# kcat/openal-soft

Hardware: AMD Instinct MI355X
Metric: mixed voices/sec @48kHz 1024-sample update, HRTF stereo; fraction of HBM roofline (higher is better)
Workload: dtype f32

## Files before the change

include/oalgpu.h:

```cpp
#ifndef OALGPU_H
#define OALGPU_H

#include <stddef.h>
#include <stdint.h>

#ifdef __cplusplus
extern "C" {
#endif
#if defined(__GNUC__)
#pragma GCC visibility push(default)
#endif

#define OALGPU_BUFFER_LINE_SIZE 1024
#define OALGPU_MAX_RESAMPLER_PADDING 48
#define OALGPU_MAX_RESAMPLER_EDGE 24
#define OALGPU_HRTF_HISTORY_LENGTH 64
#define OALGPU_HRIR_LENGTH 128
#define OALGPU_MAX_SENDS 6
#define OALGPU_MAX_OUTPUT_CHANNELS 32
#define OALGPU_MAX_AMBI_CHANNELS 25
#define OALGPU_MIXER_FRAC_BITS 16

typedef enum oalgpu_error {
    OALGPU_OK = 0,
// ... 91 lines not shown
    int32_t  hrtf;
    uint32_t max_voices;
    uint32_t max_buffers;
    uint32_t voices_per_group;
    uint32_t flags;
} oalgpu_context_desc;
#define OALGPU_CTX_FIR_VALU 1u
#define OALGPU_CTX_PROFILE  2u
#define OALGPU_CTX_STREAM_ROWS 8u
#define OALGPU_CTX_APPLY_IN_VOICE_KERNEL 16u
#define OALGPU_CTX_FUSED_REDUCE 32u
#define OALGPU_CTX_RESIDENT 64u
#define OALGPU_CTX_SLICE_LINES 128u
#define OALGPU_CTX_WAVE_PAIRS 256u
#define OALGPU_CTX_ROW_SLICES 512u
#define OALGPU_CTX_SERIAL   4u

int  oalgpu_context_create(const oalgpu_context_desc *desc, oalgpu_context **out);
void oalgpu_context_destroy(oalgpu_context *ctx);

int oalgpu_hrtf_load_mhr(oalgpu_context *ctx, const void *data, size_t size);
int oalgpu_hrtf_load_store(oalgpu_context *ctx, uint32_t sample_rate, uint32_t ir_size, const float *field_distance,
    const uint8_t *field_evcount, uint32_t num_fields, const uint16_t *elev_azcount, const uint16_t *elev_iroffset,
    uint32_t num_elevs, const float *coeffs, const uint8_t *delays, uint32_t num_irs);
typedef struct oalgpu_hrtf_info {
    uint32_t sample_rate, ir_size, num_fields, num_elevs, num_irs;
} oalgpu_hrtf_info;
int oalgpu_hrtf_info_get(oalgpu_context *ctx, oalgpu_hrtf_info *out);
int oalgpu_hrtf_raw(oalgpu_context *ctx, float *field_distance, uint8_t *field_evcount,
    uint16_t *elev_azcount, uint16_t *elev_iroffset, float *coeffs, uint8_t *delays);
// ... 352 lines not shown
```

openal-soft_amd/csrc/api.hip:

```cpp
#include "api_context.hpp"
namespace oalgpu {

thread_local std::string gLastError;

int Fail(int code, const std::string &msg)
{
    gLastError = msg;
    return code;
}

void ParkResidentContexts(int device);

int UseDevice(int device)
{
    int count = 0;
    if(hipGetDeviceCount(&count) != hipSuccess || count <= 0)
        return Fail(OALGPU_ERR_NO_DEVICE, "no HIP device available (the product has no CPU path)");
    if(device < 0 || device >= count) return Fail(OALGPU_ERR_INVALID, "device ordinal out of range");
    HIP_TRY(hipSetDevice(device));
    ParkResidentContexts(device);
    return OALGPU_OK;
}

}
// ... 212 lines not shown
    HIP_TRY(c->partHrtf.alloc(L.hrtf ? groups * (kLine + kHrirLen) * 2 : 0)); L.partHrtf = c->partHrtf.p;
    HIP_TRY(c->partHrtf2.alloc(c->useWave && L.hrtf ? groups * (kLine + kHrirLen) * 2 : 0));
    c->partHrtfBuf[0] = c->partHrtf.p; c->partHrtfBuf[1] = c->partHrtf2.p;
    HIP_TRY(c->bus.alloc(BusFloats(L))); HIP_TRY(c->bus.zero()); L.bus = c->bus.p;
    if(desc->flags & OALGPU_CTX_PROFILE)
    {
        HIP_TRY(c->phaseTimes.alloc(nv * 16)); HIP_TRY(c->phaseTimes.zero());
        c->prof.times = c->phaseTimes.p;
    }
    L.hrtfOld = nullptr; L.hrtfTgt = nullptr;

    HIP_TRY(c->dSplit.alloc(L.numDry)); HIP_TRY(c->dSplit.zero());
    HIP_TRY(c->dSplit2.alloc(L.numDry)); HIP_TRY(c->dSplit2.zero());
    HIP_TRY(c->carryBuf.alloc(size_t{kLine + kHrirLen} * 2)); HIP_TRY(c->carryBuf.zero());
    HIP_TRY(c->postArrived.alloc(1)); HIP_TRY(c->postArrived.zero());
    HIP_TRY(c->dHfScale.alloc(L.numDry)); HIP_TRY(c->dHfScale.zero());
    HIP_TRY(c->dCoeffs.alloc(size_t{L.numDry} * kHrirLen * 2)); HIP_TRY(c->dCoeffs.zero());
    HIP_TRY(c->dTemp.alloc(size_t{L.numDry} * kLine + (kLine + kHrirLen) * 2));
    if(L.rows8) SetRowsGroups(c.get());
    *out = c.release();
    return OALGPU_OK;
}

static void DetachForDestroy(oalgpu_context *ctx);

void oalgpu_context_destroy(oalgpu_context *ctx)
{
    if(!ctx) return;
    (void)UseDevice(ctx->desc.device);
    if(ctx->attachedTo || !ctx->attached.empty()) DetachForDestroy(ctx);
// ... 85 lines not shown
        }
    out[0] = st[0][0]; out[1] = st[0][1]; out[2] = st[1][1]; out[3] = st[2][2];
}

static int PostDirectHrtfFused(oalgpu_context *c, hipStream_t s, uint32_t samples_to_do, hipEvent_t evDone, bool resident = false)
{
    const DeviceLayout &L = c->L;
    float *left = L.bus + size_t{L.numDry} * kLine;
    SplitterState *spIn = c->dSplitCur ? c->dSplit2.p : c->dSplit.p, *spOut = c->dSplitCur ? c->dSplit.p : c->dSplit2.p;
    const uint32_t postEpoch = c->postEpoch + L.numDry;
    const uint32_t seg = ((samples_to_do + 63u) / 64u) | 1u;
    if(c->runPowerSeg != seg) { SplitterRunPowers(c->dSplitCoeff, seg, c->runPower); c->runPowerSeg = seg; }
    const uint32_t slot = c->outNext % oalgpu_context::kIoSlots;
    const bool ring = c->outRing && c->outFlags;
    const uint32_t outTarget = c->outArrivedTotal + PostResidentFirGroups();
    auto &R = c->res;
    if(resident)
    {
        c->reduceHeld = false;
        LaunchPostResident(s, left, left + kLine, L.bus, L.numDry, L.bus + BusAccumOffset(L), c->carryBuf.p, spIn, spOut, c->dHfScale.p, c->dCoeffs.p,
            c->dIrSize, samples_to_do, c->dTemp.p, c->postArrived.p, postEpoch, c->runPower, evDone, ring ? c->outHost[slot] : nullptr,
            ring ? c->outFlags + size_t{slot} * 16 : nullptr, c->outSeq + 1u, R.counters.p, R.hostFlags, (R.posts + 1u) * R.redGroups,
            (R.posts + 1u) * R.firGroups, R.posts + 1u);
        HIP_TRY(hipGetLastError());
        ++R.posts;
    }
    else if(c->reduceHeld)
    {
        c->reduceHeld = false;
        if(!c->reducedCount.p) { HIP_TRY(c->reducedCount.alloc(1)); HIP_TRY(c->reducedCount.zero()); }
        const uint32_t reducedEpoch = c->reducedEpoch + ReducePostReduceGroups(c->heldL);
        LaunchReducePostFused(s, c->heldL, CarrySource(c, c->carryAccum && L.hrtf), left, left + kLine, L.bus, L.numDry, L.bus + BusAccumOffset(L),
            c->carryBuf.p, spIn, spOut, c->dHfScale.p, c->dCoeffs.p, c->dIrSize, samples_to_do, c->dTemp.p, c->postArrived.p, postEpoch,
            c->runPower, evDone, ring ? c->outHost[slot] : nullptr, ring ? c->outFlags + size_t{slot} * 16 : nullptr, c->outSeq + 1u,
            c->outArrived.p, outTarget, c->reducedCount.p, reducedEpoch);
        HIP_TRY(hipGetLastError());
        c->reducedEpoch = reducedEpoch;
        if(ring) c->outArrivedTotal = outTarget;
    }
    else
    {
        LaunchPostDirectHrtfFused(s, left, left + kLine, L.bus, L.numDry, L.bus + BusAccumOffset(L), c->carryBuf.p, spIn, spOut,
            c->dHfScale.p, c->dCoeffs.p, c->dIrSize, samples_to_do, c->dTemp.p, c->postArrived.p, postEpoch, c->runPower, evDone,
            ring ? c->outHost[slot] : nullptr, ring ? c->outFlags + size_t{slot} * 16 : nullptr, c->outSeq + 1u, c->outArrived.p, outTarget);
        HIP_TRY(hipGetLastError());
        if(ring) c->outArrivedTotal = outTarget;
    }
    c->postEpoch = postEpoch;
    if(ring) c->outSlotSeq[slot] = ++c->outSeq;
    c->outRingWritten = ring;
    c->dSplitCur ^= 1u;
    c->carryInBuf = true;
    return OALGPU_OK;
}

int JoinPost(oalgpu_context *c)
{
    if(!c->postPending) return OALGPU_OK;
    HIP_TRY(hipStreamWaitEvent(c->stream, c->lastPostEvent ? c->lastPostEvent : c->evPostDone, 0));
// ... 787 lines not shown
```

openal-soft_amd/csrc/api_context.hpp:

```cpp
#pragma once
#include "../../include/oalgpu.h"
#ifdef OALGPU_MEASUREMENT
#include "../../tools/measure/oalgpu_measure.h"
#endif

#include <hip/hip_runtime.h>
#include <hip/hip_ext.h>
#include <rccl/rccl.h>
#include <dlfcn.h>
#include <fcntl.h>
#include <sys/mman.h>
#include <sys/stat.h>
#include <unistd.h>

#include <algorithm>
#include <atomic>
#include <chrono>
#include <functional>
#include <thread>
#include <cstdio>
#include <cstdlib>
#include <cstring>
#include <memory>
#include <mutex>
// ... 169 lines not shown
    DevBuf<float> cfState;
    uint32_t distLines{0};
    DevBuf<uint32_t> distDelays;
    DevBuf<float> distGains, distHist;
    DevBuf<unsigned char> pcm;
    DevBuf<float> hFieldDist, hCoeffs;
    DevBuf<uint8_t> hEvCount, hDelays;
    DevBuf<uint16_t> hAzCount, hIrOffset;
    DevBuf<SplitterState> dSplit, dSplit2;
    uint32_t dSplitCur{0};
    DevBuf<float> carryBuf;
    float dSplitCoeff{0.0f};
    float runPower[4]{1.0f, 0.0f, 1.0f, 1.0f};
    uint32_t runPowerSeg{0};
    DevBuf<uint32_t> postArrived;
    uint32_t postEpoch{0};
    const ParamRecord *nextRecs{nullptr};
    const int32_t *nextMap{nullptr};
    const float *nextRows{nullptr};
    bool carryInBuf{false};
    DevBuf<float> dHfScale, dCoeffs, dTemp;
    uint32_t dIrSize{0};
    bool directSet{false};
    DevBuf<ParamRecord> paramDev;
    std::vector<ParamRecord> paramHost;
    DevBuf<VoiceInitRecord> initDev;
    std::vector<VoiceInitRecord> initPending;
    struct CbVoice {
        uint32_t voice{0}; int32_t buffer{-1}; uint32_t frameBytes{4}, capacityFrames{0};
        oalgpu_callback_fn fn{nullptr}; void *user{nullptr};
// ... 119 lines not shown
```

openal-soft_amd/csrc/kernels.hpp:

```cpp
#pragma once
#include <hip/hip_runtime.h>
#include <stdint.h>

#include "dev_hrtf.hpp"
#include "dev_mix.hpp"
#include "dev_resample.hpp"
#include "dev_voice.hpp"
#include "../host/limiter_params.hpp"
#include "../host/uhj_params.hpp"
#include "../host/stabilizer_params.hpp"
#include "../host/crossfeed_params.hpp"

namespace oalgpu {

enum VoiceFlagBits : uint32_t {
    kFlagFading = 1u << 0,
    kFlagHasHrtf = 1u << 1,
    kFlagDirectFilter = 1u << 2,
    kFlagHrtfDirty = 1u << 3,
    kFlagAmbiScale = 1u << 4,
    kFlagNfc = 1u << 5,
    kFlagQueue = 1u << 7,
    kFlagDelayed = 1u << 6,
    kFlagSendFilterShift = 8
// ... 199 lines not shown
void LaunchMixDirectHrtf(hipStream_t s, bool exact, float *left, float *right, const float *in, uint32_t nch,
    float *accum, SplitterState *splitters, const float *hfscales, const float *chanCoeffs, uint32_t irsize,
    uint32_t n, float *temp);
void LaunchBiquadDual(hipStream_t s, BiquadState *f0, BiquadState *f1, const float *src, float *dst, uint32_t n);
void LaunchGetCoeffs(hipStream_t s, const HrtfStoreDev &st, const float *dirs, uint32_t count, float *coeffs,
    uint32_t *delays);

void LaunchPostDirectHrtfFast(hipStream_t s, float *left, float *right, const float *in, uint32_t nch, float *accum,
    SplitterState *splitters, const float *hfscales, const float *chanCoeffs, uint32_t irsize, uint32_t n, float *temp,
    hipEvent_t evDone = nullptr);

inline uint32_t ReducePostReduceGroups(const DeviceLayout &L) { return uint32_t((BusFloats(L) + 63u) / 64u); }
void LaunchReducePostFused(hipStream_t s, const DeviceLayout &L, const float *carry, float *left, float *right, const float *in, uint32_t nch,
    const float *accIn, float *carryOut, const SplitterState *spIn, SplitterState *spOut, const float *hfscales, const float *chanCoeffs,
    uint32_t irsize, uint32_t n, float *xf, uint32_t *arrived, uint32_t epoch, const float runPower[4], hipEvent_t evDone,
    float *hostOut, uint32_t *hostFlag, uint32_t hostSeq, uint32_t *outArrived, uint32_t outTarget, uint32_t *reduced, uint32_t reducedEpoch);
void LaunchPostDirectHrtfFused(hipStream_t s, float *left, float *right, const float *in, uint32_t nch, const float *accIn, float *carryOut,
    const SplitterState *spIn, SplitterState *spOut, const float *hfscales, const float *chanCoeffs, uint32_t irsize, uint32_t n,
    float *xf, uint32_t *arrived, uint32_t epoch, const float runPower[4], hipEvent_t evDone = nullptr,
    float *hostOut = nullptr, uint32_t *hostFlag = nullptr, uint32_t hostSeq = 0, uint32_t *outArrived = nullptr, uint32_t outTarget = 0);
void LaunchBusReduceResident(hipStream_t s, const DeviceLayout &L, const float *carry, uint32_t *counters, uint32_t *hostFlags, uint32_t set,
    uint32_t arriveTarget, uint32_t postDoneTarget);
uint32_t PostResidentFirGroups();
void LaunchPostResident(hipStream_t s, float *left, float *right, const float *in, uint32_t nch, const float *accIn, float *carryOut,
    const SplitterState *spIn, SplitterState *spOut, const float *hfscales, const float *chanCoeffs, uint32_t irsize, uint32_t n,
    float *xf, uint32_t *arrived, uint32_t epoch, const float runPower[4], hipEvent_t evDone, float *hostOut, uint32_t *hostFlag, uint32_t hostSeq,
    uint32_t *counters, uint32_t *hostFlags, uint32_t redDoneTarget, uint32_t postDoneTarget, uint32_t progressValue);

void LaunchBFormatDecode(hipStream_t s, bool exact, float *out, const float *lines, SplitterState *states, float *bands,
    const float *gainsHf, const float *gainsLf, uint32_t nin, uint32_t nout, uint32_t n);
void LaunchDither(hipStream_t s, float *lines, uint32_t nlines, uint32_t n, float quantScale, uint32_t seed);
uint32_t DitherAdvanceSeed(uint32_t seed, uint32_t draws);
void LaunchWriteSamples(hipStream_t s, int sampleType, const float *lines, uint32_t nlines, uint32_t n, uint32_t frameStep, void *out);
void LaunchLimiter(hipStream_t s, float *lines, uint32_t n, const LimiterConsts &k, float *state);
size_t LimiterStateFloats(uint32_t nch);
constexpr size_t kLimiterHoldHistory = 16u + 1024u;
void LaunchUhjEncode(hipStream_t s, int quality, float *left, float *right, const float *w, const float *x, const float *y,
    uint32_t n, const float *taps, float *state);
size_t UhjStateFloats(int quality);
void LaunchTsmeEncode(hipStream_t s, int quality, float *left, float *right, const float *dry, uint32_t n, const float *taps,
    float *state);
constexpr size_t kStabilizerScratch = 64;
// ... 141 lines not shown
```

openal-soft_amd/csrc/post_wave.hip:

```cpp
#include <hip/hip_ext.h>
#include "dev_wave.hpp"
#include "dev_reduce.hpp"

#pragma clang fp contract(off)

namespace oalgpu {
namespace {

constexpr int kPostFrames = kLine + kHrirLen;
constexpr int kPostGroup = 4;

__global__ void OALGPU_SINGLE_DS_OPS __launch_bounds__(64) __attribute__((amdgpu_num_vgpr(32))) PostSplitKernel(const float *__restrict__ in, float *__restrict__ xf,
    SplitterState *__restrict__ splitters, const float *__restrict__ hfscales, uint32_t n)
{
    __shared__ float x[kLine + 64];
    const uint32_t c = blockIdx.x, lane = threadIdx.x;
    for(uint32_t k = lane; k < uint32_t(kLine); k += 64) x[k] = (k < n) ? in[size_t{c} * kLine + k] : 0.0f;
    WaveSync();
    SplitterState st = splitters[c];
    SplitterScanHfTri(st, x, n, hfscales[c], lane);
    if(lane == 0) splitters[c] = st;
    WaveSync();
    for(uint32_t k = lane; k < uint32_t(kLine); k += 64) xf[size_t{c} * kLine + k] = (k < n) ? x[k] : 0.0f;
}
// ... 70 lines not shown
    {
        const uint32_t o = t + 256u * uint32_t(k);
        if(o >= n && o < n + kHrirLen && o < uint32_t(kPostFrames)) accOut[o - n] = tot[k];
    }
    __syncthreads();
#pragma unroll
    for(int k = 0; k < kPer; ++k)
    {
        const uint32_t o = t + 256u * uint32_t(k);
        if(o >= uint32_t(kHrirLen) && o < kHrirLen + n && o < uint32_t(kPostFrames)) accOut[o] = f2{0.0f, 0.0f};
    }
}

__device__ __forceinline__ void PostStoreCoherent(float *p, float v) { __hip_atomic_store(p, v, __ATOMIC_RELAXED, __HIP_MEMORY_SCOPE_AGENT); }
__device__ __forceinline__ float PostLoadCoherent(const float *p) { return __hip_atomic_load(p, __ATOMIC_RELAXED, __HIP_MEMORY_SCOPE_AGENT); }

constexpr int kFusedFrames = 64;

template<class F>
__device__ __forceinline__ bool PostWait(F ready, int nap, uint32_t *waited = nullptr)
{
    if(ready()) return true;
    const unsigned long long t0 = __builtin_amdgcn_s_memrealtime();
    bool ok = false;
    for(uint32_t spins = 0;; ++spins)
    {
        if(nap <= 4) __builtin_amdgcn_s_sleep(4); else __builtin_amdgcn_s_sleep(8);
        if(ready()) { ok = true; break; }
        if((spins & 63u) == 63u && __builtin_amdgcn_s_memrealtime() - t0 > kResidentWatchdogTicks) break;
    }
    if(waited) __hip_atomic_fetch_add(waited, uint32_t(__builtin_amdgcn_s_memrealtime() - t0), __ATOMIC_RELAXED, __HIP_MEMORY_SCOPE_AGENT);
    return ok;
}
__device__ __forceinline__ bool PostWaitCounter(const uint32_t *counter, uint32_t target, int nap, uint32_t *waited = nullptr)
{
    return PostWait([&]() { return int32_t(__hip_atomic_load(counter, __ATOMIC_RELAXED, __HIP_MEMORY_SCOPE_AGENT) - target) >= 0; }, nap, waited);
}
struct PostResident { uint32_t *postDone; uint32_t postDoneTarget; uint32_t *progress; uint32_t progressValue; uint32_t *error; uint32_t *counters; };
template<int MODE>
__device__ __forceinline__ void PostFusedBlock(float *xs, uint32_t wg, uint32_t tid, uint32_t outTarget, const float *__restrict__ in, uint32_t nch,
    const SplitterState *__restrict__ spIn, SplitterState *__restrict__ spOut, const float *__restrict__ hfscales,
    const float *__restrict__ chanCoeffs, uint32_t taps, const float *__restrict__ accIn, float *__restrict__ carryOut,
    float *__restrict__ left, float *__restrict__ right, uint32_t n, float *__restrict__ xf, uint32_t *__restrict__ arrived, uint32_t epoch,
    Tri3 runPower, float *__restrict__ hostOut, uint32_t *__restrict__ hostFlag, uint32_t hostSeq, uint32_t *__restrict__ outArrived,
    const uint32_t *__restrict__ reduced, uint32_t reducedEpoch, PostResident PR = PostResident{nullptr, 0u, nullptr, 0u, nullptr, nullptr})
{
    constexpr bool FUSED = MODE != 0, RESID = MODE == 2;
    const uint32_t lane = tid;
    if(wg < nch)
    {
        const uint32_t c = wg;
        if constexpr (FUSED)
        {
            if(!PostWaitCounter(reduced, reducedEpoch, 4, (RESID && wg == 0 && lane == 0) ? PR.counters + 16u * kRcWaitRedDone : nullptr) && PR.error && lane == 0) __hip_atomic_store(PR.error, 1u, __ATOMIC_RELAXED, __HIP_MEMORY_SCOPE_SYSTEM);
#pragma unroll 8
            for(uint32_t k = lane; k < uint32_t(kLine); k += 64) xs[k] = (k < n) ? PostLoadCoherent(in + size_t{c} * kLine + k) : 0.0f;
        }
        else
        {
#pragma unroll 8
            for(uint32_t k = lane; k < uint32_t(kLine); k += 64) xs[k] = (k < n) ? in[size_t{c} * kLine + k] : 0.0f;
        }
        WaveSync();
        SplitterState st = spIn[c];
        SplitterScanHfDpp(st, xs, n, hfscales[c], lane, runPower);
        if(lane == 0) spOut[c] = st;
        WaveSync();
#pragma unroll 8
        for(uint32_t k = lane; k < uint32_t(kLine); k += 64) PostStoreCoherent(xf + size_t{c} * kLine + k, (k < n) ? xs[k] : 0.0f);
        asm volatile("s_waitcnt vmcnt(0)" ::: "memory");
        if(lane == 0) __hip_atomic_fetch_add(arrived, 1u, __ATOMIC_RELAXED, __HIP_MEMORY_SCOPE_AGENT);
        return;
    }
    const uint32_t blk = wg - nch;
    const uint32_t o = blk * uint32_t(kFusedFrames) + lane;
    const int32_t base = int32_t(blk) * kFusedFrames - kHrirLen;
    constexpr int kCoefDw = kHrirLen * 2;
    constexpr int kWin = kHrirLen + kFusedFrames;
    constexpr int kPair = 2;
// ... 4 lines not shown
    {
        typedef const __attribute__((address_space(1))) float *gfloatp;
        gfloatp src = reinterpret_cast<gfloatp>((const __attribute__((address_space(1))) void*)(chanCoeffs + size_t{c0} * kCoefDw)) + lane;
        float *dst = cst + lane;
#pragma unroll 1
        for(uint32_t q = 0; q < gc; ++q)
        {
            const float a = src[0], b = src[64], c2 = src[128], d = src[192];
            dst[0] = a; dst[64] = b; dst[128] = c2; dst[192] = d;
            src += kCoefDw; dst += kCoefDw;
        }
    };
    stageCoeffs(0u, nch < uint32_t(kPair) ? nch : uint32_t(kPair));
    f2 accOld = {0.0f, 0.0f};
    if constexpr (!FUSED) accOld = reinterpret_cast<const f2*>(accIn)[o];
    if(!PostWaitCounter(arrived, epoch, 8, (RESID && wg == nch && lane == 0) ? PR.counters + 16u * kRcWaitSplit : nullptr) && PR.error && lane == 0) __hip_atomic_store(PR.error, 1u, __ATOMIC_RELAXED, __HIP_MEMORY_SCOPE_SYSTEM);
    if constexpr (FUSED)
        accOld = f2{PostLoadCoherent(accIn + 2u * o), PostLoadCoherent(accIn + 2u * o + 1u)};
    float accL = 0.0f, accR = 0.0f;
    for(uint32_t c0 = 0; c0 < nch; c0 += kPair)
    {
        const uint32_t gc = (nch - c0 < uint32_t(kPair)) ? nch - c0 : uint32_t(kPair);
        WaveSync();
        if(c0) stageCoeffs(c0, gc);
        for(uint32_t c = 0; c < gc; ++c)
        {
#pragma unroll
            for(int j3 = 0; j3 < kWin / 64; ++j3)
            {
                const uint32_t j = lane + 64u * uint32_t(j3);
                const int32_t fr = base + int32_t(j);
                xw4[c][j] = (fr >= 0 && fr < kLine) ? PostLoadCoherent(xf + size_t{c0 + c} * kLine + uint32_t(fr)) : 0.0f;
            }
        }
        WaveSync();
        for(uint32_t c = 0; c < gc; ++c)
        {
            const float *xw = &xw4[c][kHrirLen + lane];
            const f2 *cw = reinterpret_cast<const f2*>(cst + c * uint32_t(kCoefDw));
#pragma unroll 1
            for(uint32_t t4 = 0; t4 < taps; t4 += 4)
            {
                float x[4]; f2 cc[4];
#pragma unroll
                for(int j = 0; j < 4; ++j) { x[j] = xw[-int32_t(t4) - j]; cc[j] = cw[t4 + uint32_t(j)]; }
#pragma unroll
                for(int j = 0; j < 4; ++j)
                {
                    accL = __builtin_fmaf(cc[j].x, x[j], accL);
                    accR = __builtin_fmaf(cc[j].y, x[j], accR);
                }
            }
// ... 48 lines not shown
        {
            const uint32_t t = __hip_atomic_fetch_add(outArrived, 1u, __ATOMIC_ACQ_REL, __HIP_MEMORY_SCOPE_AGENT);
            if(t + 1u == outTarget)
            {
                __threadfence_system();
                __hip_atomic_store(hostFlag, hostSeq, __ATOMIC_RELEASE, __HIP_MEMORY_SCOPE_SYSTEM);
            }
        }
    }
}

__global__ void OALGPU_SINGLE_DS_OPS __launch_bounds__(64) __attribute__((amdgpu_num_vgpr(48))) PostFusedKernel(const float *__restrict__ in, uint32_t nch,
    const SplitterState *__restrict__ spIn, SplitterState *__restrict__ spOut, const float *__restrict__ hfscales,
    const float *__restrict__ chanCoeffs, uint32_t taps, const float *__restrict__ accIn, float *__restrict__ carryOut,
    float *__restrict__ left, float *__restrict__ right, uint32_t n, float *__restrict__ xf, uint32_t *__restrict__ arrived, uint32_t epoch,
    Tri3 runPower, float *__restrict__ hostOut, uint32_t *__restrict__ hostFlag, uint32_t hostSeq, uint32_t *__restrict__ outArrived, uint32_t outTarget)
{
    __shared__ float xs[kLine + 64];
    __builtin_amdgcn_s_setprio(3);
    PostFusedBlock<0>(xs, blockIdx.x, threadIdx.x, outTarget, in, nch, spIn, spOut, hfscales, chanCoeffs, taps, accIn, carryOut, left, right, n,
        xf, arrived, epoch, runPower, hostOut, hostFlag, hostSeq, outArrived, nullptr, 0u);
}

#ifndef OALGPU_FUSED_KF
#define OALGPU_FUSED_KF 4
#endif
struct ReducePostArgs {
    const float *carry; uint32_t nReduce;
    const float *in; uint32_t nch;
    const SplitterState *spIn; SplitterState *spOut; const float *hfscales, *chanCoeffs; uint32_t taps;
    const float *accIn; float *carryOut, *left, *right; uint32_t n; float *xf; uint32_t *arrived; uint32_t epoch; Tri3 runPower;
    float *hostOut; uint32_t *hostFlag; uint32_t hostSeq; uint32_t *outArrived; uint32_t outTarget;
    uint32_t *reduced; uint32_t reducedEpoch;
};
__global__ void OALGPU_SINGLE_DS_OPS __launch_bounds__(256) __attribute__((amdgpu_num_vgpr(48))) ReducePostFusedKernel(DeviceLayout L, ReducePostArgs A)
{
    __shared__ float xs[kLine + 64];
    if(blockIdx.x < A.nReduce)
    {
        BusReduceBlock<4, true, OALGPU_FUSED_KF>(L, A.carry, reinterpret_cast<float (*)[64]>(xs), blockIdx.x, threadIdx.x);
        if(threadIdx.x < 64)
        {
            asm volatile("s_waitcnt vmcnt(0)" ::: "memory");
            if(threadIdx.x == 0) __hip_atomic_fetch_add(A.reduced, 1u, __ATOMIC_RELAXED, __HIP_MEMORY_SCOPE_AGENT);
        }
        return;
    }
    if(threadIdx.x >= 64) return;
    PostFusedBlock<1>(xs, blockIdx.x - A.nReduce, threadIdx.x, A.outTarget, A.in, A.nch, A.spIn, A.spOut, A.hfscales, A.chanCoeffs, A.taps,
        A.accIn, A.carryOut, A.left, A.right, A.n, A.xf, A.arrived, A.epoch, A.runPower, A.hostOut, A.hostFlag, A.hostSeq, A.outArrived, A.reduced, A.reducedEpoch);
}

struct ResidentReduceArgs {
    uint32_t *counters, *hostFlags;
    uint32_t set, arriveTarget, postDoneTarget;
};
__global__ void __launch_bounds__(256) __attribute__((amdgpu_num_vgpr(48))) BusReduceResidentKernel(DeviceLayout L, const float *__restrict__ carry,
    ResidentReduceArgs A)
{
    __shared__ float slice[4][64];
    const uint32_t tid = threadIdx.x;
    __builtin_amdgcn_s_setprio(3);
    if(tid == 0)
    {
        if(!PostWaitCounter(A.counters + 16u * (kRcArrive0 + A.set), A.arriveTarget, 4, blockIdx.x == 0 ? A.counters + 16u * kRcWaitArrive : nullptr))
            __hip_atomic_store(A.hostFlags + 16u * kRhError, 2u, __ATOMIC_RELAXED, __HIP_MEMORY_SCOPE_SYSTEM);
    }
    __syncthreads();
    auto mid = [&]()
    {
        asm volatile("s_waitcnt vmcnt(0)" ::: "memory");
        __syncthreads();
        if(tid == 0)
        {
            __hip_atomic_fetch_add(A.counters + 16u * kRcRedRead, 1u, __ATOMIC_RELAXED, __HIP_MEMORY_SCOPE_AGENT);
            if(!PostWaitCounter(A.counters + 16u * kRcPostDone, A.postDoneTarget, 4, blockIdx.x == 0 ? A.counters + 16u * kRcWaitPost : nullptr))
                __hip_atomic_store(A.hostFlags + 16u * kRhError, 3u, __ATOMIC_RELAXED, __HIP_MEMORY_SCOPE_SYSTEM);
        }
        __syncthreads();
    };
    BusReduceBlock<4, true, 8, true>(L, carry, slice, blockIdx.x, tid, mid);
    if(tid < 64)
    {
        asm volatile("s_waitcnt vmcnt(0)" ::: "memory");
        if(tid == 0) __hip_atomic_fetch_add(A.counters + 16u * kRcRedDone, 1u, __ATOMIC_RELAXED, __HIP_MEMORY_SCOPE_AGENT);
    }
}

__global__ void OALGPU_SINGLE_DS_OPS __launch_bounds__(64) __attribute__((amdgpu_num_vgpr(48))) PostResidentKernel(const float *__restrict__ in, uint32_t nch,
    const SplitterState *__restrict__ spIn, SplitterState *__restrict__ spOut, const float *__restrict__ hfscales,
    const float *__restrict__ chanCoeffs, uint32_t taps, const float *__restrict__ accIn, float *__restrict__ carryOut,
    float *__restrict__ left, float *__restrict__ right, uint32_t n, float *__restrict__ xf, uint32_t *__restrict__ arrived, uint32_t epoch,
    Tri3 runPower, float *__restrict__ hostOut, uint32_t *__restrict__ hostFlag, uint32_t hostSeq, const uint32_t *__restrict__ reduced,
    uint32_t reducedEpoch, PostResident PR)
{
    __shared__ float xs[kLine + 64];
    __builtin_amdgcn_s_setprio(3);
    PostFusedBlock<2>(xs, blockIdx.x, threadIdx.x, 0u, in, nch, spIn, spOut, hfscales, chanCoeffs, taps, accIn, carryOut, left, right, n,
        xf, arrived, epoch, runPower, hostOut, hostFlag, hostSeq, nullptr, reduced, reducedEpoch, PR);
}

}

void LaunchBusReduceResident(hipStream_t s, const DeviceLayout &L, const float *carry, uint32_t *counters, uint32_t *hostFlags, uint32_t set,
    uint32_t arriveTarget, uint32_t postDoneTarget)
{
    const uint32_t total = uint32_t(BusFloats(L));
    hipLaunchKernelGGL(BusReduceResidentKernel, dim3((total + 63u) / 64u), dim3(256), 0, s, L, carry, ResidentReduceArgs{counters, hostFlags, set, arriveTarget, postDoneTarget});
}

uint32_t PostResidentFirGroups() { return uint32_t(kPostFrames / kFusedFrames); }
void LaunchPostResident(hipStream_t s, float *left, float *right, const float *in, uint32_t nch, const float *accIn, float *carryOut,
    const SplitterState *spIn, SplitterState *spOut, const float *hfscales, const float *chanCoeffs, uint32_t irsize, uint32_t n,
    float *xf, uint32_t *arrived, uint32_t epoch, const float runPower[4], hipEvent_t evDone, float *hostOut, uint32_t *hostFlag, uint32_t hostSeq,
    uint32_t *counters, uint32_t *hostFlags, uint32_t redDoneTarget, uint32_t postDoneTarget, uint32_t progressValue)
{
    const uint32_t taps = irsize <= 16u ? 16u : ((irsize + 15u) & ~15u);
    const Tri3 P{runPower[0], runPower[1], runPower[2], runPower[3]};
    const PostResident PR{counters + 16u * kRcPostDone, postDoneTarget, hostFlags + 16u * kRhProgress, progressValue, hostFlags + 16u * kRhError, counters};
    hipExtLaunchKernelGGL(PostResidentKernel, dim3(nch + kPostFrames / kFusedFrames), dim3(64), 0, s, nullptr, evDone, 0u, in, nch, spIn, spOut, hfscales,
        chanCoeffs, taps, accIn, carryOut, left, right, n, xf, arrived, epoch, P, hostOut, hostFlag, hostSeq, counters + 16u * kRcRedDone, redDoneTarget, PR);
}

void LaunchPostDirectHrtfFused(hipStream_t s, float *left, float *right, const float *in, uint32_t nch, const float *accIn, float *carryOut,
    const SplitterState *spIn, SplitterState *spOut, const float *hfscales, const float *chanCoeffs, uint32_t irsize, uint32_t n,
    float *xf, uint32_t *arrived, uint32_t epoch, const float runPower[4], hipEvent_t evDone,
    float *hostOut, uint32_t *hostFlag, uint32_t hostSeq, uint32_t *outArrived, uint32_t outTarget)
{
    const uint32_t taps = irsize <= 16u ? 16u : ((irsize + 15u) & ~15u);
    const Tri3 P{runPower[0], runPower[1], runPower[2], runPower[3]};
    static_assert(kPostFrames % kFusedFrames == 0, "whole workgroups");
    hipExtLaunchKernelGGL(PostFusedKernel, dim3(nch + kPostFrames / kFusedFrames), dim3(64), 0, s, nullptr, evDone, 0u, in, nch, spIn, spOut, hfscales,
        chanCoeffs, taps, accIn, carryOut, left, right, n, xf, arrived, epoch, P, hostOut, hostFlag, hostSeq, outArrived, outTarget);
}

void LaunchReducePostFused(hipStream_t s, const DeviceLayout &L, const float *carry, float *left, float *right, const float *in, uint32_t nch,
    const float *accIn, float *carryOut, const SplitterState *spIn, SplitterState *spOut, const float *hfscales, const float *chanCoeffs,
    uint32_t irsize, uint32_t n, float *xf, uint32_t *arrived, uint32_t epoch, const float runPower[4], hipEvent_t evDone,
    float *hostOut, uint32_t *hostFlag, uint32_t hostSeq, uint32_t *outArrived, uint32_t outTarget, uint32_t *reduced, uint32_t reducedEpoch)
{
    ReducePostArgs A{};
    A.carry = carry; A.nReduce = ReducePostReduceGroups(L);
    A.in = in; A.nch = nch; A.spIn = spIn; A.spOut = spOut; A.hfscales = hfscales; A.chanCoeffs = chanCoeffs;
    A.taps = irsize <= 16u ? 16u : ((irsize + 15u) & ~15u);
    A.accIn = accIn; A.carryOut = carryOut; A.left = left; A.right = right; A.n = n; A.xf = xf; A.arrived = arrived; A.epoch = epoch;
    A.runPower = Tri3{runPower[0], runPower[1], runPower[2], runPower[3]};
    A.hostOut = hostOut; A.hostFlag = hostFlag; A.hostSeq = hostSeq; A.outArrived = outArrived; A.outTarget = outTarget; A.reduced = reduced; A.reducedEpoch = reducedEpoch;
    hipExtLaunchKernelGGL(ReducePostFusedKernel, dim3(A.nReduce + nch + kPostFrames / kFusedFrames), dim3(256), 0, s, nullptr, evDone, 0u, L, A);
}

void LaunchPostDirectHrtfFast(hipStream_t s, float *left, float *right, const float *in, uint32_t nch, float *accum,
    SplitterState *splitters, const float *hfscales, const float *chanCoeffs, uint32_t irsize, uint32_t n, float *temp, hipEvent_t evDone)
{
    float *xf = temp, *tmp = temp + size_t{nch} * kLine;
    const uint32_t taps = irsize <= 16u ? 16u : ((irsize + 15u) & ~15u);
    hipLaunchKernelGGL(PostSplitKernel, dim3(nch), dim3(64), 0, s, in, xf, splitters, hfscales, n);
    hipLaunchKernelGGL(PostFirKernel<16>, dim3(kPostFrames / 16), dim3(64), 0, s, xf, nch, chanCoeffs, taps, tmp);
    hipExtLaunchKernelGGL(PostShiftKernel, dim3(1), dim3(256), 0, s, nullptr, evDone, 0u, left, right, accum, tmp, n);
}

}
```

openal-soft_amd/oalgpu/__init__.py:

```python
import ctypes as C
import os

import numpy as np

PKG_DIR = os.path.dirname(os.path.dirname(os.path.abspath(__file__)))
LIB_PATH = os.path.join(PKG_DIR, "liboalgpu.so")

BUFFER_LINE = 1024
MAX_PAD = 48
HRTF_HIST = 64
HRIR_LEN = 128
MAX_SENDS = 6
(OUT_I8, OUT_U8, OUT_I16, OUT_U16, OUT_I32, OUT_U32, OUT_F32) = range(7)
MAX_OUT = 32
MAX_AMBI = 25
MATH_EXACT, MATH_FAST = 0, 1
(RS_POINT, RS_LINEAR, RS_SPLINE, RS_GAUSSIAN, RS_FAST_BSINC12, RS_BSINC12, RS_FAST_BSINC24,
 RS_BSINC24, RS_FAST_BSINC48, RS_BSINC48) = range(10)
FMT_UBYTE, FMT_SHORT, FMT_INT, FMT_FLOAT, FMT_DOUBLE, FMT_MULAW, FMT_ALAW = range(7)
FMT_DTYPES = {FMT_UBYTE: np.uint8, FMT_SHORT: np.int16, FMT_INT: np.int32, FMT_FLOAT: np.float32,
              FMT_DOUBLE: np.float64, FMT_MULAW: np.uint8, FMT_ALAW: np.uint8}
VOICE_STOPPED, VOICE_PLAYING, VOICE_STOPPING, VOICE_PENDING = range(4)

f32p = C.POINTER(C.c_float)
# ... 40 lines not shown
                ("num_aux_sends", C.c_uint32), ("num_slots", C.c_uint32),
                ("wet_channels", C.c_uint32), ("hrtf", C.c_int32), ("max_voices", C.c_uint32),
                ("max_buffers", C.c_uint32), ("voices_per_group", C.c_uint32), ("flags", C.c_uint32)]


class VoiceEvent(C.Structure):
    _fields_ = [("voice", C.c_uint32), ("play_state", C.c_int32), ("has_buffer", C.c_int32), ("current_buffer", C.c_int32),
                ("buffers_done", C.c_uint32), ("position", C.c_int32), ("position_frac", C.c_uint32), ("fading", C.c_int32)]


CTX_FIR_VALU, CTX_PROFILE, CTX_SERIAL, CTX_STREAM_ROWS, CTX_APPLY_IN_VOICE_KERNEL, CTX_FUSED_REDUCE = 1, 2, 4, 8, 16, 32
CTX_RESIDENT = 64
CTX_SLICE_LINES = 128
CTX_WAVE_PAIRS = 256
CTX_ROW_SLICES = 512


class VoiceDesc(C.Structure):
    _fields_ = [("buffer", C.c_int32), ("looping", C.c_int32), ("position", C.c_int32),
                ("position_frac", C.c_uint32), ("frequency", C.c_uint32)]


class FilterParams(C.Structure):
    _fields_ = [("active", C.c_int32), ("gain_hf", C.c_float), ("hf_norm", C.c_float),
                ("gain_lf", C.c_float), ("lf_norm", C.c_float)]


class VoiceParams(C.Structure):
    _fields_ = [("step", C.c_uint32), ("resampler", C.c_int32), ("direct_filter", FilterParams),
                ("dry_gains", C.c_float * MAX_OUT),
# ... 967 lines not shown
```

Baseline: 112.8 million.

## Skip splitter and HRTF FIR for silent ambisonic channels in post pass

```diff
diff --git a/include/oalgpu.h b/include/oalgpu.h
--- a/include/oalgpu.h
+++ b/include/oalgpu.h
@@ -129,6 +129,7 @@
 #define OALGPU_CTX_SLICE_LINES 128u
 #define OALGPU_CTX_WAVE_PAIRS 256u
 #define OALGPU_CTX_ROW_SLICES 512u
+#define OALGPU_CTX_POST_NO_SILENCE_SKIP 1024u
 #define OALGPU_CTX_SERIAL   4u
 
 int  oalgpu_context_create(const oalgpu_context_desc *desc, oalgpu_context **out);
diff --git a/openal-soft_amd/csrc/api.hip b/openal-soft_amd/csrc/api.hip
--- a/openal-soft_amd/csrc/api.hip
+++ b/openal-soft_amd/csrc/api.hip
@@ -250,6 +250,7 @@
     HIP_TRY(c->dSplit2.alloc(L.numDry)); HIP_TRY(c->dSplit2.zero());
     HIP_TRY(c->carryBuf.alloc(size_t{kLine + kHrirLen} * 2)); HIP_TRY(c->carryBuf.zero());
     HIP_TRY(c->postArrived.alloc(1)); HIP_TRY(c->postArrived.zero());
+    HIP_TRY(c->postSilent.alloc(L.numDry)); HIP_TRY(c->postSilent.zero());
     HIP_TRY(c->dHfScale.alloc(L.numDry)); HIP_TRY(c->dHfScale.zero());
     HIP_TRY(c->dCoeffs.alloc(size_t{L.numDry} * kHrirLen * 2)); HIP_TRY(c->dCoeffs.zero());
     HIP_TRY(c->dTemp.alloc(size_t{L.numDry} * kLine + (kLine + kHrirLen) * 2));
@@ -365,6 +366,7 @@
     const uint32_t slot = c->outNext % oalgpu_context::kIoSlots;
     const bool ring = c->outRing && c->outFlags;
     const uint32_t outTarget = c->outArrivedTotal + PostResidentFirGroups();
+    uint32_t *silent = (c->desc.flags & OALGPU_CTX_POST_NO_SILENCE_SKIP) ? nullptr : c->postSilent.p;
     auto &R = c->res;
     if(resident)
     {
@@ -372,7 +374,7 @@
         LaunchPostResident(s, left, left + kLine, L.bus, L.numDry, L.bus + BusAccumOffset(L), c->carryBuf.p, spIn, spOut, c->dHfScale.p, c->dCoeffs.p,
             c->dIrSize, samples_to_do, c->dTemp.p, c->postArrived.p, postEpoch, c->runPower, evDone, ring ? c->outHost[slot] : nullptr,
             ring ? c->outFlags + size_t{slot} * 16 : nullptr, c->outSeq + 1u, R.counters.p, R.hostFlags, (R.posts + 1u) * R.redGroups,
-            (R.posts + 1u) * R.firGroups, R.posts + 1u);
+            (R.posts + 1u) * R.firGroups, R.posts + 1u, silent);
         HIP_TRY(hipGetLastError());
         ++R.posts;
     }
@@ -384,7 +386,7 @@
         LaunchReducePostFused(s, c->heldL, CarrySource(c, c->carryAccum && L.hrtf), left, left + kLine, L.bus, L.numDry, L.bus + BusAccumOffset(L),
             c->carryBuf.p, spIn, spOut, c->dHfScale.p, c->dCoeffs.p, c->dIrSize, samples_to_do, c->dTemp.p, c->postArrived.p, postEpoch,
             c->runPower, evDone, ring ? c->outHost[slot] : nullptr, ring ? c->outFlags + size_t{slot} * 16 : nullptr, c->outSeq + 1u,
-            c->outArrived.p, outTarget, c->reducedCount.p, reducedEpoch);
+            c->outArrived.p, outTarget, c->reducedCount.p, reducedEpoch, silent);
         HIP_TRY(hipGetLastError());
         c->reducedEpoch = reducedEpoch;
         if(ring) c->outArrivedTotal = outTarget;
@@ -393,7 +395,7 @@
     {
         LaunchPostDirectHrtfFused(s, left, left + kLine, L.bus, L.numDry, L.bus + BusAccumOffset(L), c->carryBuf.p, spIn, spOut,
             c->dHfScale.p, c->dCoeffs.p, c->dIrSize, samples_to_do, c->dTemp.p, c->postArrived.p, postEpoch, c->runPower, evDone,
-            ring ? c->outHost[slot] : nullptr, ring ? c->outFlags + size_t{slot} * 16 : nullptr, c->outSeq + 1u, c->outArrived.p, outTarget);
+            ring ? c->outHost[slot] : nullptr, ring ? c->outFlags + size_t{slot} * 16 : nullptr, c->outSeq + 1u, c->outArrived.p, outTarget, silent);
         HIP_TRY(hipGetLastError());
         if(ring) c->outArrivedTotal = outTarget;
     }
diff --git a/openal-soft_amd/csrc/api_context.hpp b/openal-soft_amd/csrc/api_context.hpp
--- a/openal-soft_amd/csrc/api_context.hpp
+++ b/openal-soft_amd/csrc/api_context.hpp
@@ -207,6 +207,7 @@
     float runPower[4]{1.0f, 0.0f, 1.0f, 1.0f};
     uint32_t runPowerSeg{0};
     DevBuf<uint32_t> postArrived;
+    DevBuf<uint32_t> postSilent;
     uint32_t postEpoch{0};
     const ParamRecord *nextRecs{nullptr};
     const int32_t *nextMap{nullptr};
diff --git a/openal-soft_amd/csrc/kernels.hpp b/openal-soft_amd/csrc/kernels.hpp
--- a/openal-soft_amd/csrc/kernels.hpp
+++ b/openal-soft_amd/csrc/kernels.hpp
@@ -237,18 +237,20 @@
 void LaunchReducePostFused(hipStream_t s, const DeviceLayout &L, const float *carry, float *left, float *right, const float *in, uint32_t nch,
     const float *accIn, float *carryOut, const SplitterState *spIn, SplitterState *spOut, const float *hfscales, const float *chanCoeffs,
     uint32_t irsize, uint32_t n, float *xf, uint32_t *arrived, uint32_t epoch, const float runPower[4], hipEvent_t evDone,
-    float *hostOut, uint32_t *hostFlag, uint32_t hostSeq, uint32_t *outArrived, uint32_t outTarget, uint32_t *reduced, uint32_t reducedEpoch);
+    float *hostOut, uint32_t *hostFlag, uint32_t hostSeq, uint32_t *outArrived, uint32_t outTarget, uint32_t *reduced, uint32_t reducedEpoch,
+    uint32_t *silent);
 void LaunchPostDirectHrtfFused(hipStream_t s, float *left, float *right, const float *in, uint32_t nch, const float *accIn, float *carryOut,
     const SplitterState *spIn, SplitterState *spOut, const float *hfscales, const float *chanCoeffs, uint32_t irsize, uint32_t n,
     float *xf, uint32_t *arrived, uint32_t epoch, const float runPower[4], hipEvent_t evDone = nullptr,
-    float *hostOut = nullptr, uint32_t *hostFlag = nullptr, uint32_t hostSeq = 0, uint32_t *outArrived = nullptr, uint32_t outTarget = 0);
+    float *hostOut = nullptr, uint32_t *hostFlag = nullptr, uint32_t hostSeq = 0, uint32_t *outArrived = nullptr, uint32_t outTarget = 0,
+    uint32_t *silent = nullptr);
 void LaunchBusReduceResident(hipStream_t s, const DeviceLayout &L, const float *carry, uint32_t *counters, uint32_t *hostFlags, uint32_t set,
     uint32_t arriveTarget, uint32_t postDoneTarget);
 uint32_t PostResidentFirGroups();
 void LaunchPostResident(hipStream_t s, float *left, float *right, const float *in, uint32_t nch, const float *accIn, float *carryOut,
     const SplitterState *spIn, SplitterState *spOut, const float *hfscales, const float *chanCoeffs, uint32_t irsize, uint32_t n,
     float *xf, uint32_t *arrived, uint32_t epoch, const float runPower[4], hipEvent_t evDone, float *hostOut, uint32_t *hostFlag, uint32_t hostSeq,
-    uint32_t *counters, uint32_t *hostFlags, uint32_t redDoneTarget, uint32_t postDoneTarget, uint32_t progressValue);
+    uint32_t *counters, uint32_t *hostFlags, uint32_t redDoneTarget, uint32_t postDoneTarget, uint32_t progressValue, uint32_t *silent);
 
 void LaunchBFormatDecode(hipStream_t s, bool exact, float *out, const float *lines, SplitterState *states, float *bands,
     const float *gainsHf, const float *gainsLf, uint32_t nin, uint32_t nout, uint32_t n);
diff --git a/openal-soft_amd/csrc/post_wave.hip b/openal-soft_amd/csrc/post_wave.hip
--- a/openal-soft_amd/csrc/post_wave.hip
+++ b/openal-soft_amd/csrc/post_wave.hip
@@ -108,27 +108,30 @@
 
 __device__ __forceinline__ void PostStoreCoherent(float *p, float v) { __hip_atomic_store(p, v, __ATOMIC_RELAXED, __HIP_MEMORY_SCOPE_AGENT); }
 __device__ __forceinline__ float PostLoadCoherent(const float *p) { return __hip_atomic_load(p, __ATOMIC_RELAXED, __HIP_MEMORY_SCOPE_AGENT); }
+__device__ __forceinline__ void PostStoreCoherent(uint32_t *p, uint32_t v) { __hip_atomic_store(p, v, __ATOMIC_RELAXED, __HIP_MEMORY_SCOPE_AGENT); }
+__device__ __forceinline__ uint32_t PostLoadCoherent(const uint32_t *p) { return __hip_atomic_load(p, __ATOMIC_RELAXED, __HIP_MEMORY_SCOPE_AGENT); }
 
 constexpr int kFusedFrames = 64;
 
 template<class F>
-__device__ __forceinline__ bool PostWait(F ready, int nap, uint32_t *waited = nullptr)
+__device__ __forceinline__ bool PostWait(F ready, int nap, uint32_t *waited = nullptr, bool patient = false)
 {
     if(ready()) return true;
     const unsigned long long t0 = __builtin_amdgcn_s_memrealtime();
     bool ok = false;
     for(uint32_t spins = 0;; ++spins)
     {
-        if(nap <= 4) __builtin_amdgcn_s_sleep(4); else __builtin_amdgcn_s_sleep(8);
+        if(patient && spins >= 16u) __builtin_amdgcn_s_sleep(32);
+        else if(nap <= 4) __builtin_amdgcn_s_sleep(4); else __builtin_amdgcn_s_sleep(8);
         if(ready()) { ok = true; break; }
         if((spins & 63u) == 63u && __builtin_amdgcn_s_memrealtime() - t0 > kResidentWatchdogTicks) break;
     }
     if(waited) __hip_atomic_fetch_add(waited, uint32_t(__builtin_amdgcn_s_memrealtime() - t0), __ATOMIC_RELAXED, __HIP_MEMORY_SCOPE_AGENT);
     return ok;
 }
-__device__ __forceinline__ bool PostWaitCounter(const uint32_t *counter, uint32_t target, int nap, uint32_t *waited = nullptr)
-{
-    return PostWait([&]() { return int32_t(__hip_atomic_load(counter, __ATOMIC_RELAXED, __HIP_MEMORY_SCOPE_AGENT) - target) >= 0; }, nap, waited);
+__device__ __forceinline__ bool PostWaitCounter(const uint32_t *counter, uint32_t target, int nap, uint32_t *waited = nullptr, bool patient = false)
+{
+    return PostWait([&]() { return int32_t(__hip_atomic_load(counter, __ATOMIC_RELAXED, __HIP_MEMORY_SCOPE_AGENT) - target) >= 0; }, nap, waited, patient);
 }
 struct PostResident { uint32_t *postDone; uint32_t postDoneTarget; uint32_t *progress; uint32_t progressValue; uint32_t *error; uint32_t *counters; };
 template<int MODE>
@@ -137,26 +140,49 @@
     const float *__restrict__ chanCoeffs, uint32_t taps, const float *__restrict__ accIn, float *__restrict__ carryOut,
     float *__restrict__ left, float *__restrict__ right, uint32_t n, float *__restrict__ xf, uint32_t *__restrict__ arrived, uint32_t epoch,
     Tri3 runPower, float *__restrict__ hostOut, uint32_t *__restrict__ hostFlag, uint32_t hostSeq, uint32_t *__restrict__ outArrived,
-    const uint32_t *__restrict__ reduced, uint32_t reducedEpoch, PostResident PR = PostResident{nullptr, 0u, nullptr, 0u, nullptr, nullptr})
+    const uint32_t *__restrict__ reduced, uint32_t reducedEpoch, uint32_t *__restrict__ silent,
+    PostResident PR = PostResident{nullptr, 0u, nullptr, 0u, nullptr, nullptr})
 {
     constexpr bool FUSED = MODE != 0, RESID = MODE == 2;
     const uint32_t lane = tid;
     if(wg < nch)
     {
         const uint32_t c = wg;
+        uint32_t mag = 0u;
         if constexpr (FUSED)
         {
-            if(!PostWaitCounter(reduced, reducedEpoch, 4, (RESID && wg == 0 && lane == 0) ? PR.counters + 16u * kRcWaitRedDone : nullptr) && PR.error && lane == 0) __hip_atomic_store(PR.error, 1u, __ATOMIC_RELAXED, __HIP_MEMORY_SCOPE_SYSTEM);
+            if(!PostWaitCounter(reduced, reducedEpoch, 4, (RESID && wg == 0 && lane == 0) ? PR.counters + 16u * kRcWaitRedDone : nullptr, RESID) && PR.error && lane == 0) __hip_atomic_store(PR.error, 1u, __ATOMIC_RELAXED, __HIP_MEMORY_SCOPE_SYSTEM);
 #pragma unroll 8
-            for(uint32_t k = lane; k < uint32_t(kLine); k += 64) xs[k] = (k < n) ? PostLoadCoherent(in + size_t{c} * kLine + k) : 0.0f;
+            for(uint32_t k = lane; k < uint32_t(kLine); k += 64)
+            {
+                const float v = (k < n) ? PostLoadCoherent(in + size_t{c} * kLine + k) : 0.0f;
+                xs[k] = v; mag |= __builtin_bit_cast(uint32_t, v);
+            }
         }
         else
         {
 #pragma unroll 8
-            for(uint32_t k = lane; k < uint32_t(kLine); k += 64) xs[k] = (k < n) ? in[size_t{c} * kLine + k] : 0.0f;
+            for(uint32_t k = lane; k < uint32_t(kLine); k += 64)
+            {
+                const float v = (k < n) ? in[size_t{c} * kLine + k] : 0.0f;
+                xs[k] = v; mag |= __builtin_bit_cast(uint32_t, v);
+            }
         }
         WaveSync();
         SplitterState st = spIn[c];
+        if(silent)
+        {
+            mag |= __builtin_bit_cast(uint32_t, st.lpZ1) | __builtin_bit_cast(uint32_t, st.lpZ2) | __builtin_bit_cast(uint32_t, st.apZ1);
+            const bool quiet = __builtin_amdgcn_ballot_w64((mag & 0x7fffffffu) != 0u) == 0ull;
+            if(lane == 0) PostStoreCoherent(silent + c, quiet ? epoch : ~epoch);
+            if(quiet)
+            {
+                if(lane == 0) spOut[c] = SplitterState{st.coeff, 0.0f, 0.0f, 0.0f};
+                asm volatile("s_waitcnt vmcnt(0)" ::: "memory");
+                if(lane == 0) __hip_atomic_fetch_add(arrived, 1u, __ATOMIC_RELAXED, __HIP_MEMORY_SCOPE_AGENT);
+                return;
+            }
+        }
         SplitterScanHfDpp(st, xs, n, hfscales[c], lane, runPower);
         if(lane == 0) spOut[c] = st;
         WaveSync();
@@ -191,17 +217,25 @@
     stageCoeffs(0u, nch < uint32_t(kPair) ? nch : uint32_t(kPair));
     f2 accOld = {0.0f, 0.0f};
     if constexpr (!FUSED) accOld = reinterpret_cast<const f2*>(accIn)[o];
-    if(!PostWaitCounter(arrived, epoch, 8, (RESID && wg == nch && lane == 0) ? PR.counters + 16u * kRcWaitSplit : nullptr) && PR.error && lane == 0) __hip_atomic_store(PR.error, 1u, __ATOMIC_RELAXED, __HIP_MEMORY_SCOPE_SYSTEM);
+    if(!PostWaitCounter(arrived, epoch, 8, (RESID && wg == nch && lane == 0) ? PR.counters + 16u * kRcWaitSplit : nullptr, RESID) && PR.error && lane == 0) __hip_atomic_store(PR.error, 1u, __ATOMIC_RELAXED, __HIP_MEMORY_SCOPE_SYSTEM);
     if constexpr (FUSED)
         accOld = f2{PostLoadCoherent(accIn + 2u * o), PostLoadCoherent(accIn + 2u * o + 1u)};
+    uint32_t quietMask = 0u;
+    if(silent)
+    {
+        const uint32_t tag = (lane < nch) ? PostLoadCoherent(silent + lane) : ~epoch;
+        quietMask = uint32_t(__builtin_amdgcn_ballot_w64(tag == epoch));
+    }
     float accL = 0.0f, accR = 0.0f;
     for(uint32_t c0 = 0; c0 < nch; c0 += kPair)
     {
         const uint32_t gc = (nch - c0 < uint32_t(kPair)) ? nch - c0 : uint32_t(kPair);
+        if(((quietMask >> c0) & ((1u << gc) - 1u)) == ((1u << gc) - 1u)) continue;
         WaveSync();
         if(c0) stageCoeffs(c0, gc);
         for(uint32_t c = 0; c < gc; ++c)
         {
+            if((quietMask >> (c0 + c)) & 1u) continue;
 #pragma unroll
             for(int j3 = 0; j3 < kWin / 64; ++j3)
             {
@@ -213,6 +247,7 @@
         WaveSync();
         for(uint32_t c = 0; c < gc; ++c)
         {
+            if((quietMask >> (c0 + c)) & 1u) continue;
             const float *xw = &xw4[c][kHrirLen + lane];
             const f2 *cw = reinterpret_cast<const f2*>(cst + c * uint32_t(kCoefDw));
 #pragma unroll 1
@@ -291,12 +326,13 @@
     const SplitterState *__restrict__ spIn, SplitterState *__restrict__ spOut, const float *__restrict__ hfscales,
     const float *__restrict__ chanCoeffs, uint32_t taps, const float *__restrict__ accIn, float *__restrict__ carryOut,
     float *__restrict__ left, float *__restrict__ right, uint32_t n, float *__restrict__ xf, uint32_t *__restrict__ arrived, uint32_t epoch,
-    Tri3 runPower, float *__restrict__ hostOut, uint32_t *__restrict__ hostFlag, uint32_t hostSeq, uint32_t *__restrict__ outArrived, uint32_t outTarget)
+    Tri3 runPower, float *__restrict__ hostOut, uint32_t *__restrict__ hostFlag, uint32_t hostSeq, uint32_t *__restrict__ outArrived, uint32_t outTarget,
+    uint32_t *__restrict__ silent)
 {
     __shared__ float xs[kLine + 64];
     __builtin_amdgcn_s_setprio(3);
     PostFusedBlock<0>(xs, blockIdx.x, threadIdx.x, outTarget, in, nch, spIn, spOut, hfscales, chanCoeffs, taps, accIn, carryOut, left, right, n,
-        xf, arrived, epoch, runPower, hostOut, hostFlag, hostSeq, outArrived, nullptr, 0u);
+        xf, arrived, epoch, runPower, hostOut, hostFlag, hostSeq, outArrived, nullptr, 0u, silent);
 }
 
 #ifndef OALGPU_FUSED_KF
@@ -308,7 +344,7 @@
     const SplitterState *spIn; SplitterState *spOut; const float *hfscales, *chanCoeffs; uint32_t taps;
     const float *accIn; float *carryOut, *left, *right; uint32_t n; float *xf; uint32_t *arrived; uint32_t epoch; Tri3 runPower;
     float *hostOut; uint32_t *hostFlag; uint32_t hostSeq; uint32_t *outArrived; uint32_t outTarget;
-    uint32_t *reduced; uint32_t reducedEpoch;
+    uint32_t *reduced; uint32_t reducedEpoch; uint32_t *silent;
 };
 __global__ void OALGPU_SINGLE_DS_OPS __launch_bounds__(256) __attribute__((amdgpu_num_vgpr(48))) ReducePostFusedKernel(DeviceLayout L, ReducePostArgs A)
 {
@@ -325,7 +361,7 @@
     }
     if(threadIdx.x >= 64) return;
     PostFusedBlock<1>(xs, blockIdx.x - A.nReduce, threadIdx.x, A.outTarget, A.in, A.nch, A.spIn, A.spOut, A.hfscales, A.chanCoeffs, A.taps,
-        A.accIn, A.carryOut, A.left, A.right, A.n, A.xf, A.arrived, A.epoch, A.runPower, A.hostOut, A.hostFlag, A.hostSeq, A.outArrived, A.reduced, A.reducedEpoch);
+        A.accIn, A.carryOut, A.left, A.right, A.n, A.xf, A.arrived, A.epoch, A.runPower, A.hostOut, A.hostFlag, A.hostSeq, A.outArrived, A.reduced, A.reducedEpoch, A.silent);
 }
 
 struct ResidentReduceArgs {
@@ -340,7 +376,7 @@
     __builtin_amdgcn_s_setprio(3);
     if(tid == 0)
     {
-        if(!PostWaitCounter(A.counters + 16u * (kRcArrive0 + A.set), A.arriveTarget, 4, blockIdx.x == 0 ? A.counters + 16u * kRcWaitArrive : nullptr))
+        if(!PostWaitCounter(A.counters + 16u * (kRcArrive0 + A.set), A.arriveTarget, 4, blockIdx.x == 0 ? A.counters + 16u * kRcWaitArrive : nullptr, true))
             __hip_atomic_store(A.hostFlags + 16u * kRhError, 2u, __ATOMIC_RELAXED, __HIP_MEMORY_SCOPE_SYSTEM);
     }
     __syncthreads();
@@ -351,7 +387,7 @@
         if(tid == 0)
         {
             __hip_atomic_fetch_add(A.counters + 16u * kRcRedRead, 1u, __ATOMIC_RELAXED, __HIP_MEMORY_SCOPE_AGENT);
-            if(!PostWaitCounter(A.counters + 16u * kRcPostDone, A.postDoneTarget, 4, blockIdx.x == 0 ? A.counters + 16u * kRcWaitPost : nullptr))
+            if(!PostWaitCounter(A.counters + 16u * kRcPostDone, A.postDoneTarget, 4, blockIdx.x == 0 ? A.counters + 16u * kRcWaitPost : nullptr, true))
                 __hip_atomic_store(A.hostFlags + 16u * kRhError, 3u, __ATOMIC_RELAXED, __HIP_MEMORY_SCOPE_SYSTEM);
         }
         __syncthreads();
@@ -369,12 +405,12 @@
     const float *__restrict__ chanCoeffs, uint32_t taps, const float *__restrict__ accIn, float *__restrict__ carryOut,
     float *__restrict__ left, float *__restrict__ right, uint32_t n, float *__restrict__ xf, uint32_t *__restrict__ arrived, uint32_t epoch,
     Tri3 runPower, float *__restrict__ hostOut, uint32_t *__restrict__ hostFlag, uint32_t hostSeq, const uint32_t *__restrict__ reduced,
-    uint32_t reducedEpoch, PostResident PR)
+    uint32_t reducedEpoch, PostResident PR, uint32_t *__restrict__ silent)
 {
     __shared__ float xs[kLine + 64];
     __builtin_amdgcn_s_setprio(3);
     PostFusedBlock<2>(xs, blockIdx.x, threadIdx.x, 0u, in, nch, spIn, spOut, hfscales, chanCoeffs, taps, accIn, carryOut, left, right, n,
-        xf, arrived, epoch, runPower, hostOut, hostFlag, hostSeq, nullptr, reduced, reducedEpoch, PR);
+        xf, arrived, epoch, runPower, hostOut, hostFlag, hostSeq, nullptr, reduced, reducedEpoch, silent, PR);
 }
 
 }
@@ -390,31 +426,31 @@
 void LaunchPostResident(hipStream_t s, float *left, float *right, const float *in, uint32_t nch, const float *accIn, float *carryOut,
     const SplitterState *spIn, SplitterState *spOut, const float *hfscales, const float *chanCoeffs, uint32_t irsize, uint32_t n,
     float *xf, uint32_t *arrived, uint32_t epoch, const float runPower[4], hipEvent_t evDone, float *hostOut, uint32_t *hostFlag, uint32_t hostSeq,
-    uint32_t *counters, uint32_t *hostFlags, uint32_t redDoneTarget, uint32_t postDoneTarget, uint32_t progressValue)
+    uint32_t *counters, uint32_t *hostFlags, uint32_t redDoneTarget, uint32_t postDoneTarget, uint32_t progressValue, uint32_t *silent)
 {
     const uint32_t taps = irsize <= 16u ? 16u : ((irsize + 15u) & ~15u);
     const Tri3 P{runPower[0], runPower[1], runPower[2], runPower[3]};
     const PostResident PR{counters + 16u * kRcPostDone, postDoneTarget, hostFlags + 16u * kRhProgress, progressValue, hostFlags + 16u * kRhError, counters};
     hipExtLaunchKernelGGL(PostResidentKernel, dim3(nch + kPostFrames / kFusedFrames), dim3(64), 0, s, nullptr, evDone, 0u, in, nch, spIn, spOut, hfscales,
-        chanCoeffs, taps, accIn, carryOut, left, right, n, xf, arrived, epoch, P, hostOut, hostFlag, hostSeq, counters + 16u * kRcRedDone, redDoneTarget, PR);
+        chanCoeffs, taps, accIn, carryOut, left, right, n, xf, arrived, epoch, P, hostOut, hostFlag, hostSeq, counters + 16u * kRcRedDone, redDoneTarget, PR, silent);
 }
 
 void LaunchPostDirectHrtfFused(hipStream_t s, float *left, float *right, const float *in, uint32_t nch, const float *accIn, float *carryOut,
     const SplitterState *spIn, SplitterState *spOut, const float *hfscales, const float *chanCoeffs, uint32_t irsize, uint32_t n,
     float *xf, uint32_t *arrived, uint32_t epoch, const float runPower[4], hipEvent_t evDone,
-    float *hostOut, uint32_t *hostFlag, uint32_t hostSeq, uint32_t *outArrived, uint32_t outTarget)
+    float *hostOut, uint32_t *hostFlag, uint32_t hostSeq, uint32_t *outArrived, uint32_t outTarget, uint32_t *silent)
 {
     const uint32_t taps = irsize <= 16u ? 16u : ((irsize + 15u) & ~15u);
     const Tri3 P{runPower[0], runPower[1], runPower[2], runPower[3]};
     static_assert(kPostFrames % kFusedFrames == 0, "whole workgroups");
     hipExtLaunchKernelGGL(PostFusedKernel, dim3(nch + kPostFrames / kFusedFrames), dim3(64), 0, s, nullptr, evDone, 0u, in, nch, spIn, spOut, hfscales,
-        chanCoeffs, taps, accIn, carryOut, left, right, n, xf, arrived, epoch, P, hostOut, hostFlag, hostSeq, outArrived, outTarget);
+        chanCoeffs, taps, accIn, carryOut, left, right, n, xf, arrived, epoch, P, hostOut, hostFlag, hostSeq, outArrived, outTarget, silent);
 }
 
 void LaunchReducePostFused(hipStream_t s, const DeviceLayout &L, const float *carry, float *left, float *right, const float *in, uint32_t nch,
     const float *accIn, float *carryOut, const SplitterState *spIn, SplitterState *spOut, const float *hfscales, const float *chanCoeffs,
     uint32_t irsize, uint32_t n, float *xf, uint32_t *arrived, uint32_t epoch, const float runPower[4], hipEvent_t evDone,
-    float *hostOut, uint32_t *hostFlag, uint32_t hostSeq, uint32_t *outArrived, uint32_t outTarget, uint32_t *reduced, uint32_t reducedEpoch)
+    float *hostOut, uint32_t *hostFlag, uint32_t hostSeq, uint32_t *outArrived, uint32_t outTarget, uint32_t *reduced, uint32_t reducedEpoch, uint32_t *silent)
 {
     ReducePostArgs A{};
     A.carry = carry; A.nReduce = ReducePostReduceGroups(L);
@@ -422,7 +458,7 @@
     A.taps = irsize <= 16u ? 16u : ((irsize + 15u) & ~15u);
     A.accIn = accIn; A.carryOut = carryOut; A.left = left; A.right = right; A.n = n; A.xf = xf; A.arrived = arrived; A.epoch = epoch;
     A.runPower = Tri3{runPower[0], runPower[1], runPower[2], runPower[3]};
-    A.hostOut = hostOut; A.hostFlag = hostFlag; A.hostSeq = hostSeq; A.outArrived = outArrived; A.outTarget = outTarget; A.reduced = reduced; A.reducedEpoch = reducedEpoch;
+    A.hostOut = hostOut; A.hostFlag = hostFlag; A.hostSeq = hostSeq; A.outArrived = outArrived; A.outTarget = outTarget; A.reduced = reduced; A.reducedEpoch = reducedEpoch; A.silent = silent;
     hipExtLaunchKernelGGL(ReducePostFusedKernel, dim3(A.nReduce + nch + kPostFrames / kFusedFrames), dim3(256), 0, s, nullptr, evDone, 0u, L, A);
 }
 
diff --git a/openal-soft_amd/oalgpu/__init__.py b/openal-soft_amd/oalgpu/__init__.py
--- a/openal-soft_amd/oalgpu/__init__.py
+++ b/openal-soft_amd/oalgpu/__init__.py
@@ -78,6 +78,7 @@
 CTX_SLICE_LINES = 128
 CTX_WAVE_PAIRS = 256
 CTX_ROW_SLICES = 512
+CTX_POST_NO_SILENCE_SKIP = 1024
 
 
 class VoiceDesc(C.Structure):
```

Measured after the change: 112.1 million. Within noise of the previous version (-0.6%).
